# 5l1v3r1/PBS

Hardware: AMD Instinct MI355X
Metric: co-run slowdown (%) vs solo + aggregate throughput, 4-tenant mix at 1/2/4/8 GPU (higher is better)
Workload: dtype bf16

## Files before the change

csrc/hip/common.hpp:

```cpp
#pragma once
#include <hip/hip_runtime.h>

#include <cstdint>
#include <cstdio>
#include <cstdlib>

namespace gpbs_hip {

constexpr int kXcds = 8;
constexpr int kMaxTenants = 64;
constexpr int kNumPmc = 4;
constexpr uint32_t kNoOwner = 0xFFFFFFFFu;
constexpr uint32_t kSplitBit = 0x80000000u;
constexpr uint32_t kOwnerMask = 0x7FFFFFFFu;

typedef __bf16 bf16x8 __attribute__((ext_vector_type(8)));
typedef float f32x4 __attribute__((ext_vector_type(4)));
typedef float f32x16 __attribute__((ext_vector_type(16)));
typedef unsigned int u32x4 __attribute__((ext_vector_type(4)));
typedef unsigned int u32x2 __attribute__((ext_vector_type(2)));
typedef unsigned short u16;
typedef unsigned int u32;
typedef unsigned long long u64;

// ... 88 lines not shown
    const u32 se = se_id();
    const u32* w = t->owner + kCtx * (xcc & 7) + se;
    const u32 o = (mode & GATE_DEVTABLE) ? __hip_atomic_load(w, __ATOMIC_RELAXED, __HIP_MEMORY_SCOPE_AGENT)
                                         : __hip_atomic_load(w, __ATOMIC_RELAXED, __HIP_MEMORY_SCOPE_SYSTEM);
    return (o & kOwnerMask) == me;
  }
  const u64* q = t->pair[xcc & 7];
  const u64 p01 = (mode & GATE_DEVTABLE) ? __hip_atomic_load(q, __ATOMIC_RELAXED, __HIP_MEMORY_SCOPE_AGENT)
                                         : __hip_atomic_load(q, __ATOMIC_RELAXED, __HIP_MEMORY_SCOPE_SYSTEM);
  const u32 w0 = (u32)p01, w1 = (u32)(p01 >> 32);
  const bool h0 = (w0 & kOwnerMask) == me, h1 = (w1 & kOwnerMask) == me;
  if (!(mode & GATE_SPATIAL) || (h0 && h1)) {
    if (h0 || h1) return true;
    const u64 p23 = (mode & GATE_DEVTABLE) ? __hip_atomic_load(q + 1, __ATOMIC_RELAXED, __HIP_MEMORY_SCOPE_AGENT)
                                           : __hip_atomic_load(q + 1, __ATOMIC_RELAXED, __HIP_MEMORY_SCOPE_SYSTEM);
    return (u32)p23 == me || (u32)(p23 >> 32) == me;
  }
  if (h0) return !(w0 & kSplitBit) || cu_half() == 0;
  if (h1) return !(w1 & kSplitBit) || cu_half() == 1;
  return false;
}

__device__ __forceinline__ void count(u64* cnt, u32 me, u32 xcc, u64 inst, u64 cyc, u64 refs, u64 miss) {
  if (!cnt) return;
  u64* c = cnt + ((size_t)me * kXcds + (xcc & 7)) * kNumPmc;
  if (inst) __hip_atomic_fetch_add(c + 0, inst, __ATOMIC_RELAXED, __HIP_MEMORY_SCOPE_SYSTEM);
  if (cyc) __hip_atomic_fetch_add(c + 1, cyc, __ATOMIC_RELAXED, __HIP_MEMORY_SCOPE_SYSTEM);
  if (refs) __hip_atomic_fetch_add(c + 2, refs, __ATOMIC_RELAXED, __HIP_MEMORY_SCOPE_SYSTEM);
  if (miss) __hip_atomic_fetch_add(c + 3, miss, __ATOMIC_RELAXED, __HIP_MEMORY_SCOPE_SYSTEM);
}
// ... 40 lines not shown
```

csrc/hip/runtime.cpp:

```cpp
#include <hip/hip_runtime.h>
#include <hsa/hsa.h>
#include <hsa/hsa_ext_amd.h>
#include <rocprofiler-sdk-roctx/roctx.h>
#include <x86intrin.h>

#include <algorithm>
#include <atomic>
#include <cmath>
#include <cstdio>
#include <cstdlib>
#include <chrono>
#include <condition_variable>
#include <cstring>
#include <deque>
#include <memory>
#include <mutex>
#include <thread>
#include <vector>

#include "../include/gpbs/gpbs.h"
#include "common.hpp"
#include "hwc_attr.h"

using namespace gpbs_hip;

extern "C" {
int gpbs_adapt_update(gpbs_adapt_state_t*, const gpbs_adapt_params_t*, uint64_t, uint64_t, uint64_t, uint64_t);
int gpbs_hip_gemm_units(int, int);
int gpbs_hip_gemm_fp8_units(int, int);
int gpbs_hwc_sample(uint64_t* out, int nxcd);
int gpbs_hwc_sample_se(uint64_t* se_out, uint64_t* x_out);
int gpbs_hwc_slot_per_se(int k);
int gpbs_hwc_active(void);
int gpbs_hip_gemm_bf16(const void*, const void*, void*, int, int, int, void*, const void*, unsigned, unsigned, void*,
                       void*, int, hipStream_t);
int gpbs_hip_gemm_fp8(const void*, const float*, const void*, const float*, void*, int, int, int, int, void*, const void*,
                      unsigned, unsigned, void*, void*, int, hipStream_t);
int gpbs_hip_stream_copy(const void*, void*, unsigned long long, unsigned, void*, const void*, unsigned, unsigned,
                         void*, void*, int, hipStream_t);
int gpbs_hip_reduce_bf16(const void*, const void*, void*, unsigned long long, unsigned, void*, const void*, unsigned,
                         unsigned, void*, void*, int, hipStream_t);
int gpbs_hip_gemv_bf16(const void*, const void*, void*, int, int, void*, const void*, unsigned, unsigned, void*, void*,
                       int, hipStream_t);
int gpbs_hip_partition_switch(void*, unsigned, const unsigned*, hipStream_t);
int gpbs_hip_counter_reduce(void*, void*, const int*, int, void*, hipStream_t);
int gpbs_hip_adapt(void*, const void*, const void*, const void*, int, const gpbs_adapt_params_t*, int*, hipStream_t);
int gpbs_hip_switch_probe(const void*, int, unsigned*, int, unsigned, unsigned long long, hipStream_t);
int gpbs_hip_hwc_attribute(const void*, void*, void*, void*, hipStream_t);
// ... 1128 lines not shown
        (!B || X.gen > B->gen))
      B = &X;
  if (!B) return -22;
  if (hipEventQuery(B->ev) != hipSuccess) {
    B->state = 2;
    c->async_late++;
    return -11;
  }
  std::memcpy(states_out, B->st, sizeof(gpbs_adapt_state_t) * max);
  std::memcpy(tenants_out, B->ids, sizeof(int) * max);
  B->state = 0;
  return max;
}


enum Kind { K_GEMM = 1, K_STREAM = 2, K_REDUCE = 3, K_GEMV = 4, K_ALLREDUCE = 5, K_GEMM_FP8 = 6 };

constexpr int kCollMax = 8;
struct CollDescHost {
  const void* in[kCollMax];
  void* out[kCollMax];
  u32* flags[kCollMax];
  u32 rank, world;
  u64 n8;
};

struct Coll {
  int device = 0, rank = 0, world = 1;
  size_t bytes = 0;
  void* in = nullptr;
// ... 6 lines not shown

}

extern "C" {

typedef struct gpbs_runner_cfg {
  int kind;
  int tenant;
  int gate;
  int priority;
  int depth;
  int grid;
  int M, N, K;
  int chunk_bytes;
  int engine_wake;
  int reserved;
  unsigned long long bytes;
  void *a, *b, *c;
  int alt_kind;
  int alt_M, alt_N, alt_K;
  int alt_chunk_bytes;
  int alt_reserved;
  unsigned long long alt_bytes;
  void *alt_a, *alt_b, *alt_c;
} gpbs_runner_cfg_t;

typedef struct gpbs_runner_stats {
  uint64_t units_done, launches, relaunches, waits_owner, submitted;
  int64_t busy_ns, wait_owner_ns, first_start_ns, last_done_ns;
  int64_t lat_sum_ns, lat_max_ns;
  uint64_t lat_count;
// ... 233 lines not shown
  std::vector<int64_t> lats;
  hipEvent_t ev[16];
  int err = 0;
  uint64_t q_hold[16] = {};

  void hold_drop(int qi) {
    if (q_hold[qi]) {
      hold_release(ctx, q_hold[qi] - 1);
      q_hold[qi] = 0;
    }
  }

  std::atomic<int> phase{0};
  uint8_t q_alt[16] = {};
  int cur_alt = 0;
  u32 q_seq[16] = {};
  u32 coll_seq = 0;
  int64_t q_t0[16] = {};

  struct Work {
    int kind, M, N, K, chunk;
    unsigned long long bytes;
    void *a, *b, *c;
  };
  static int coll_timeout_ms(const Work& w) { return w.K > 0 ? w.K : 5000; }
  Work work(int alt) const {
    if (alt && cfg.alt_kind)
      return Work{cfg.alt_kind, cfg.alt_M, cfg.alt_N, cfg.alt_K, cfg.alt_chunk_bytes, cfg.alt_bytes,
                  cfg.alt_a, cfg.alt_b, cfg.alt_c};
    return Work{cfg.kind, cfg.M, cfg.N, cfg.K, cfg.chunk_bytes, cfg.bytes, cfg.a, cfg.b, cfg.c};
  }

  static u32 unit_total(const Work& w) {
    switch (w.kind) {
      case K_ALLREDUCE: {
        const u64 n8 = w.bytes / 16, chunk8 = (u64)w.chunk / 16, per = (n8 + w.M - 1) / w.M;
        const u64 lo = (u64)w.N * per, hi = std::min(lo + per, n8);
        return hi > lo ? (u32)((hi - lo + chunk8 - 1) / chunk8) : 0u;
      }
      case K_GEMM: return (u32)gpbs_hip_gemm_units(w.M, w.N);
// ... 90 lines not shown
    const bool dev = tm != 0;
    const void* tab = tm == 1 ? (const void*)ctx->d_table : tm == 2 ? (const void*)ctx->b_table : (const void*)ctx->h_table;
    const bool gate = cfg.gate && !ctx->share.load(std::memory_order_acquire);
    const bool hold = gate && ctx->hold_enable && tm != 1 && w.kind != K_GEMV && ctx->engine &&
                      ctx->cls_cache[cfg.tenant].load(std::memory_order_relaxed) == 1;
    const unsigned mode = (gate ? (cfg.gate == 2 ? GATE_PARK : GATE_TABLE) : GATE_NONE) | (dev ? GATE_DEVTABLE : 0) |
                          (gate && ctx->spatial ? GATE_SPATIAL : 0) |
                          (gate && __atomic_load_n(&ctx->se_mode, __ATOMIC_ACQUIRE) ? GATE_SE : 0) |
                          (cfg.priority > 0 && ctx->waveprio ? GATE_WAVEPRIO : 0) | (hold ? GATE_HOLD : 0);
    const unsigned me = (unsigned)cfg.tenant;
    __atomic_store_n(&h_status[qi], 0u, __ATOMIC_RELEASE);
    st.launches++;
    const int grid = cfg.grid ? cfg.grid : cur_grid;
    switch (w.kind) {
      case K_GEMM:
        return gpbs_hip_gemm_bf16(w.a, w.b, w.c, w.M, w.N, w.K, q, tab, mode, me, ctx->d_cnt, &h_status[qi], grid,
                                  stream);
      case K_GEMM_FP8: {
        const char *aq = (const char*)w.a, *bq = (const char*)w.b;
        return gpbs_hip_gemm_fp8(aq, (const float*)(aq + (size_t)w.M * w.K), bq, (const float*)(bq + (size_t)w.N * w.K),
                                 w.c, w.M, w.N, w.K, 0, q, tab, mode, me, ctx->d_cnt, &h_status[qi], grid, stream);
      }
      case K_STREAM:
        return gpbs_hip_stream_copy(w.a, w.c, w.bytes, (unsigned)w.chunk, q, tab, mode, me, ctx->d_cnt,
                                    &h_status[qi], grid, stream);
      case K_REDUCE:
        return gpbs_hip_reduce_bf16(w.a, w.b, w.c, w.bytes, (unsigned)w.chunk, q, tab, mode, me, ctx->d_cnt,
                                    &h_status[qi], grid, stream);
      case K_GEMV:
        return gpbs_hip_gemv_bf16(w.a, w.b, w.c, w.M, w.K, q, tab, mode, me, ctx->d_cnt, &h_status[qi], grid,
                                  stream);
      case K_ALLREDUCE:
// ... 13 lines not shown

  int wo_qi = -1;
  int64_t q_l0[16] = {};
  int64_t drain_seen_rv = 0;
  int64_t ramp_from = 0;
  static void ewma(std::atomic<int64_t>& a, std::atomic<uint64_t>& n, int64_t v) {
    const int64_t o = a.load(std::memory_order_relaxed);
    a.store(n.load(std::memory_order_relaxed) ? o + (v - o) / 8 : v, std::memory_order_relaxed);
    n.fetch_add(1, std::memory_order_relaxed);
  }
  void note_drain(int qi, int64_t now) {
    if (cfg.tenant < 0 || cfg.tenant >= kMaxTenants) return;
    const int64_t rv = ctx->revoke_ns[cfg.tenant].load(std::memory_order_relaxed);
    if (!rv || rv == drain_seen_rv || rv < q_l0[qi] || now < rv) return;
    const u32 s = __atomic_load_n(&h_status[qi], __ATOMIC_ACQUIRE);
    if ((s & 0x80000000u) && (s & 0x3fffffffu) >= unit_total(work(q_alt[qi]))) return;
    drain_seen_rv = rv;
    const int64_t dr = now - rv;
    if (dr >= 1000000000) return;
    st.drain_sum_ns += dr;
    st.drain_count++;
    if (dr > st.drain_max_ns) st.drain_max_ns = dr;
    ewma(ctx->swc_drain_ns[cfg.tenant], ctx->swc_drain_n[cfg.tenant], dr);
  }
  void note_ramp(int64_t now) {
    if (!ramp_from || cfg.tenant < 0 || cfg.tenant >= kMaxTenants) return;
    const int64_t g = ctx->grant_ns[cfg.tenant].load(std::memory_order_relaxed);
    if (g >= ramp_from && now >= g && now - g < 1000000000)
      ewma(ctx->swc_ramp_ns[cfg.tenant], ctx->swc_ramp_n[cfg.tenant], now - g);
    ramp_from = 0;
  }
// ... 66 lines not shown
            if (qi < 0) break;
            fresh = true;
          }
          wo_qi = fl.empty() ? -1 : fl.front().qi;
          wait_owner();
          if (stop) break;
          if (fresh) {
            q_alt[qi] = (uint8_t)(cfg.alt_kind && phase.load(std::memory_order_acquire));
            q_seq[qi] = coll_seq++;
            q_t0[qi] = mono_ns();
          }
          cur_alt = q_alt[qi];
          hipStream_t stream = pick_stream();
          if (fresh) {
            std::lock_guard<std::mutex> g(mu);
            pending--;
            inflight++;
            next_q = (qi + 1) % nq;
            q_busy[qi] = 1;
          } else {
            relaunch.pop_front();
            st.relaunches++;
          }
          if (cfg.priority > 0 && ctx->hold_enable && fresh && !q_hold[qi]) q_hold[qi] = hold_acquire(ctx) + 1;
          q_l0[qi] = mono_ns();
          note_ramp(q_l0[qi]);
          if (launch(qi, stream) != 0) err = -5;
          const int e = qi;
          hipEventRecord(ev[e], stream);
          fl.push_back({qi, e});
        }
        if (fl.empty()) {
          std::lock_guard<std::mutex> g(mu);
          if (pending <= 0 && relaunch.empty()) break;
          continue;
        }
        Fl f = fl.front();
        fl.pop_front();
        while (hipEventQuery(ev[f.ev]) == hipErrorNotReady) {
          if (stop) break;
          std::this_thread::yield();
        }
        const u32 s = __atomic_load_n(&h_status[f.qi], __ATOMIC_ACQUIRE);
        const u32 done = s & 0x3fffffffu;
        const Work fw = work(q_alt[f.qi]);
        const bool unfinished = !((s & 0x80000000u) && done >= unit_total(fw));
        const bool coll_late = fw.kind == K_ALLREDUCE && unfinished &&
                               mono_ns() - q_t0[f.qi] > (int64_t)coll_timeout_ms(fw) * 1000000;
        if (((s & 0x80000000u) && (s & 0x40000000u)) || coll_late) {
          std::fprintf(stderr, "[gpbs-hip] tenant %d: collective unit %u timed out waiting for its peers\n",
                       cfg.tenant, q_seq[f.qi]);
          err = -110;
          hold_drop(f.qi);
          std::lock_guard<std::mutex> g(mu);
          q_busy[f.qi] = 0;
          inflight--;
          pending = 0;
          if (!submit_times.empty()) submit_times.pop_front();
        } else if ((s & 0x80000000u) && done >= unit_total(work(q_alt[f.qi]))) {
          hold_drop(f.qi);
          const int64_t t = mono_ns();
          std::lock_guard<std::mutex> g(mu);
          q_busy[f.qi] = 0;
          inflight--;
          st.units_done++;
          st.units_alt += q_alt[f.qi];
          st.last_done_ns = t;
          if (!submit_times.empty()) {
            const int64_t lat = t - submit_times.front();
            submit_times.pop_front();
            st.lat_sum_ns += lat;
            st.lat_count++;
            if (lat > st.lat_max_ns) st.lat_max_ns = lat;
            if (lats.size() < (1u << 20)) lats.push_back(lat);
          }
        } else {
          relaunch.push_back(f.qi);
          note_drain(f.qi, mono_ns());
        }
        if (stop) break;
      }
      st.busy_ns += mono_ns() - batch_t0;
      {
// ... 1377 lines not shown
      (cfg->alt_bytes % 16 || cfg->alt_chunk_bytes <= 0 || cfg->alt_chunk_bytes % 16))
    return nullptr;
  if (cfg->alt_kind == K_GEMV && cfg->alt_K % 512) return nullptr;
  if (cfg->alt_kind == K_GEMM_FP8 &&
      (cfg->alt_M <= 0 || cfg->alt_N <= 0 || cfg->alt_K <= 0 || cfg->alt_M % 128 || cfg->alt_N % 128 || cfg->alt_K % 128))
    return nullptr;
  if (cfg->alt_kind < 0 || (cfg->alt_kind > K_GEMV && cfg->alt_kind != K_GEMM_FP8)) return nullptr;
  hipSetDevice(c->device);
  for (int have = c->cnt_rows.load(); have < cfg->tenant + 1 && !c->cnt_rows.compare_exchange_weak(have, cfg->tenant + 1);) {
  }
  auto* r = new Runner;
  r->ctx = c;
  r->cfg = *cfg;
  if (r->cfg.depth <= 0) r->cfg.depth = 2;
  if (r->cfg.depth > 8) r->cfg.depth = 8;
  r->nq = r->cfg.depth + 1;
  int lo = 0, hi = 0;
  hipDeviceGetStreamPriorityRange(&lo, &hi);
  bool ok = hipStreamCreateWithPriority(&r->stream, hipStreamNonBlocking, cfg->priority ? hi : lo) == hipSuccess;
  ok = ok && hipMalloc((void**)&r->d_q, sizeof(WorkQueue) * r->nq) == hipSuccess;
  ok = ok && hipMemset(r->d_q, 0, sizeof(WorkQueue) * r->nq) == hipSuccess;
  ok = ok && hipHostMalloc((void**)&r->h_status, sizeof(u32) * r->nq, hipHostMallocCoherent | hipHostMallocMapped) ==
                 hipSuccess;
  for (int i = 0; i < r->nq && ok; ++i) ok = hipEventCreateWithFlags(&r->ev[i], hipEventDisableTiming) == hipSuccess;
  if (!ok) {
    delete r;
    return nullptr;
  }
  r->th = std::thread([r] { r->loop(); });
  return r;
}

int gpbs_runner_submit(void* p, int units) {
  Runner* r = (Runner*)p;
  const int64_t t = mono_ns();
  {
    std::lock_guard<std::mutex> g(r->mu);
    r->pending += units;
    r->st.submitted += units;
    for (int i = 0; i < units; ++i) r->submit_times.push_back(t);
  }
  r->cv.notify_all();
  return 0;
}

// ... 377 lines not shown
```

csrc/hip/tenant_kernels.hip:

```cpp
#include "common.hpp"

namespace gpbs_hip {


__device__ __forceinline__ int grab_unit_x(WorkQueue* q, const PartTable* table, u32 mode, u32 me, u32 xcc,
                                           int* s_slot, u32 total) {
  if (threadIdx.x == 0) {
    int u = -1;
    hold_wait(table, mode);
    const u32 per = (total + kXcds - 1) / kXcds;
    for (u32 spins = 0;; ++spins) {
      if (owns(table, mode, me, xcc)) {
        for (u32 k = 0; k < (u32)kXcds; ++k) {
          const u32 r = (xcc + k) & (kXcds - 1);
          const u32 lo = r * per, hi = min(lo + per, total);
          if (lo >= hi) continue;
          if (__hip_atomic_load(&q->xnext[r], __ATOMIC_RELAXED, __HIP_MEMORY_SCOPE_AGENT) >= hi - lo) continue;
          const u32 t = atomicAdd(&q->xnext[r], 1u);
          if (t < hi - lo) {
            u = (int)(lo + t);
            atomicAdd(&q->next, 1u);
            break;
          }
        }
// ... 128 lines not shown
constexpr u32 kGemmBlock2D = 1u << 17;
constexpr u32 kGemmStatic = 1u << 18;
constexpr int kGemmOptsLive = 1 | 8 | 1 << 23;
constexpr int kGemmOptsShipped = 256 | 8192 | 65536 | 131072;
static int g_gemm_opts = 8;
constexpr int kG2Half = 128 * 128;
constexpr int kG2Buf = 4 * kG2Half;
constexpr int kG2Lds = 2 * kG2Buf;

__device__ __forceinline__ int g2_swz(int r) { return (r >> 1) & 7; }

__global__ __launch_bounds__(G2_NT, 1) void k_gemm256_bf16_tn(const u16* __restrict__ A, const u16* __restrict__ Bt,
                                                             u16* __restrict__ C, int M, int N, int K, WorkQueue* q,
                                                             const PartTable* table, u32 mode, u32 me, u64* cnt,
                                                             u32 inst_per_tile, u32 refs_per_tile, u32 miss_per_tile,
                                                             u32* status) {
  __shared__ __attribute__((aligned(16))) char smem[kG2Lds + 16];
  lds_t* lds = (lds_t*)smem;
  int* s_slot = (int*)(smem + kG2Lds);
  const u32 xcc = xcc_id();
  u64 t_last = __builtin_amdgcn_s_memtime();
  const int tid = threadIdx.x, lane = tid & 63, wid = tid >> 6;
  const int wu = __builtin_amdgcn_readfirstlane(wid);
  const int wr = wu >> 2, wc = wu & 3;
  const int tiles_m = M / G2_BM, tiles_n = N / G2_BM, ntiles = tiles_m * tiles_n;
  const int nt = K / G2_BK;
  int soff[2];
#pragma unroll
  for (int j = 0; j < 2; ++j) {
    const int row = 8 * (2 * wid + j) + (lane >> 3);
    soff[j] = row * K + (((lane & 7) ^ g2_swz(row)) * 8);
  }
  int soffa[4];
#pragma unroll
  for (int j = 0; j < 4; ++j) {
    const int row = 8 * (4 * (wid & 3) + j) + (lane >> 3);
    soffa[j] = row * K + (((lane & 7) ^ g2_swz(row)) * 8);
  }
  const int l16 = lane & 15, lq = lane >> 4;
  const int bh = wc >> 1, bc = (wc & 1) * 64;
  int units_seen = 0;

  for (;;) {
    const int tile = (mode & kGemmStatic) ? (units_seen ? -1 : (int)blockIdx.x)
                     : (mode & kGemmXRange) ? grab_unit_x(q, table, mode, me, xcc, s_slot, (u32)ntiles)
                                            : grab_unit(q, table, mode, me, xcc, s_slot, (u32)ntiles);
    if (tile < 0) break;
    int tm = tile / tiles_n, tn = tile % tiles_n;
    if ((mode & kGemmBlock2D) && (tiles_m & 3) == 0 && (tiles_n & 1) == 0 && ntiles % kXcds == 0) {
      const int per = ntiles / kXcds;
      const int bm = tiles_m / 4, bn = tiles_n / 2;
      const int g = (mode & kGemmXRange) ? tile / per : tile % kXcds;
      const int jj = (mode & kGemmXRange) ? tile % per : tile / kXcds;
      tm = (g >> 1) * bm + jj / bn;
      tn = (g & 1) * bn + jj % bn;
    }
    const u16* Ab = A + (size_t)tm * G2_BM * K;
    const u16* Bb = Bt + (size_t)tn * G2_BM * K;
    auto stage = [&](int kind, int h, int t) {
      const u16* src = (kind ? Bb : Ab) + (size_t)h * 128 * K + t * G2_BK;
      lds_t* dst = lds + (t & 1) * kG2Buf + (kind * 2 + h) * kG2Half + wid * 2048;
      glds16(src + soff[0], dst);
// ... 8 lines not shown
    auto frag = [&](int b, int kind, int h, int r0, int s) -> bf16x8 {
      const int r = r0 + l16;
      const lds_t* p = lds + b * kG2Buf + (kind * 2 + h) * kG2Half + r * 128 + (((4 * s + lq) ^ g2_swz(r)) << 4);
      return *(const __attribute__((address_space(3))) bf16x8*)p;
    };
    f32x4 acc[8][4];
#pragma unroll
    for (int i = 0; i < 8; ++i)
#pragma unroll
      for (int j = 0; j < 4; ++j) acc[i][j] = f32x4{0.f, 0.f, 0.f, 0.f};
    stage(1, 0, 0); stage(1, 1, 0); stage(0, 0, 0); stage(0, 1, 0);
    asm volatile("s_waitcnt vmcnt(0)" ::: "memory");
    __builtin_amdgcn_s_barrier();
    if (wr == 1) __builtin_amdgcn_s_barrier();
    bf16x8 a[4][2], b[4][2];
    for (int t = 0; t < nt; ++t) {
      const int buf = t & 1;
      const bool more = t + 1 < nt;
#pragma unroll
      for (int j = 0; j < 4; ++j)
#pragma unroll
        for (int s2 = 0; s2 < 2; ++s2) b[j][s2] = frag(buf, 1, bh, bc + j * 16, s2);
      __builtin_amdgcn_sched_barrier(0);
#pragma unroll
      for (int i = 0; i < 4; ++i)
#pragma unroll
        for (int s2 = 0; s2 < 2; ++s2) a[i][s2] = frag(buf, 0, wr, i * 16, s2);
      if (more) {
        stage(1, 0, t + 1); stage(1, 1, t + 1);
      } else {
        asm volatile("s_waitcnt vmcnt(0)" ::: "memory");
      }
      __builtin_amdgcn_s_barrier();
      asm volatile("s_waitcnt lgkmcnt(0)" ::: "memory");
      __builtin_amdgcn_s_setprio(1);
#pragma unroll
      for (int s2 = 0; s2 < 2; ++s2)
#pragma unroll
        for (int i = 0; i < 4; ++i)
#pragma unroll
          for (int j = 0; j < 4; ++j)
            acc[i][j] = __builtin_amdgcn_mfma_f32_16x16x32_bf16(b[j][s2], a[i][s2], acc[i][j], 0, 0, 0);
      __builtin_amdgcn_s_setprio(0);
      __builtin_amdgcn_s_barrier();
#pragma unroll
      for (int i = 0; i < 4; ++i)
// ... 3 lines not shown
        stage_own_a(t + 1);
        asm volatile("s_waitcnt vmcnt(4)" ::: "memory");
      }
      __builtin_amdgcn_s_barrier();
      asm volatile("s_waitcnt lgkmcnt(0)" ::: "memory");
      __builtin_amdgcn_s_setprio(1);
#pragma unroll
      for (int s2 = 0; s2 < 2; ++s2)
#pragma unroll
        for (int i = 0; i < 4; ++i)
#pragma unroll
          for (int j = 0; j < 4; ++j)
            acc[4 + i][j] = __builtin_amdgcn_mfma_f32_16x16x32_bf16(b[j][s2], a[i][s2], acc[4 + i][j], 0, 0, 0);
      __builtin_amdgcn_s_setprio(0);
      asm volatile("s_waitcnt vmcnt(0)" ::: "memory");
      __builtin_amdgcn_s_barrier();
    }
    if (wr == 0) __builtin_amdgcn_s_barrier();
#pragma unroll
    for (int i = 0; i < 8; ++i)
#pragma unroll
      for (int j = 0; j < 4; ++j) {
        const int m = wr * 128 + i * 16 + l16;
        const int c8 = wc * 16 + j * 4 + lq;
        const u32 lo = (u32)f2bf(acc[i][j][0]) | ((u32)f2bf(acc[i][j][1]) << 16);
        const u32 hi = (u32)f2bf(acc[i][j][2]) | ((u32)f2bf(acc[i][j][3]) << 16);
        *(__attribute__((address_space(3))) u32x2*)(lds + m * 512 + ((c8 ^ (m & 15)) << 3)) = u32x2{lo, hi};
      }
    __syncthreads();
#pragma unroll
    for (int p = 0; p < 16; ++p) {
      const int row = p * 16 + (tid >> 5), c16 = tid & 31;
      u32x4 v = *(const __attribute__((address_space(3))) u32x4*)(lds + row * 512 + (((2 * c16) ^ (row & 14)) << 3));
      if (row & 1) v = u32x4{v.z, v.w, v.x, v.y};
      u32x4* dst = (u32x4*)(C + (size_t)(tm * G2_BM + row) * N + tn * G2_BM + c16 * 8);
      __builtin_nontemporal_store(v, dst);
    }
    __syncthreads();
    ++units_seen;
    if (!(mode & kGemmStatic)) count_unit(cnt, me, xcc, inst_per_tile, &t_last, refs_per_tile, miss_per_tile, q);
  }
  if (!(mode & kGemmStatic)) finish(q, status, (u32)ntiles);
}

constexpr int SNT = 256, SUNROLL = 16, RUNROLL = 6;

template <int U, bool NTS>
__global__ __launch_bounds__(SNT) void k_stream_copy(const f32x4* __restrict__ src, f32x4* __restrict__ dst,
                                                    u64 n4, u32 chunk4, WorkQueue* q, const PartTable* table, u32 mode,
                                                    u32 me, u64* cnt, u32* status) {
  __shared__ int s_slot[4];
  const u32 xcc = xcc_id();
  u64 t_last = __builtin_amdgcn_s_memtime();
  const u32 nchunks = (u32)((n4 + chunk4 - 1) / chunk4);
  const u64 lines = (u64)chunk4 * 16 / 128;
  const u64 inst = (u64)chunk4 * 2 / 64 + 8;
  for (;;) {
// ... 175 lines not shown
    warned = true;
    fprintf(stderr,
            "gpbs_hip_set_gemm_opts: bits 0x%x select GEMM variants that were removed (docs/gemm_lab.md); "
            "the shipped schedule runs\n",
            gone);
  }
  g_gemm_opts = opts & kGemmOptsLive;
  return old;
}

int gpbs_hip_gemm_units(int M, int N) {
  if (M % G2_BM == 0 && N % G2_BM == 0) return (M / G2_BM) * (N / G2_BM);
  return (M / GBM) * (N / GBN);
}

int gpbs_hip_gemm_bf16(const void* A, const void* Bt, void* C, int M, int N, int K, void* q, const void* table,
                       unsigned mode, unsigned me, void* cnt, void* status, int grid, hipStream_t s) {
  if (M % GBM || N % GBN || K % GBK || M <= 0 || N <= 0 || K <= 0) return -22;
  if (M % G2_BM == 0 && N % G2_BM == 0) {
    const int ntiles = (M / G2_BM) * (N / G2_BM);
    if (grid <= 0) grid = 256;
    if (grid > ntiles) grid = ntiles;
    const u32 inst = (u32)((G2_BM / 16) * (G2_BM / 16) * (K / 32) + (K / G2_BK) * 64 + 128);
    const u32 refs = (u32)(((u64)2 * G2_BM * K * 2) / 128);
    const u32 miss = (u32)((((u64)M + N) * K * 2 / 128) / ntiles + (u64)G2_BM * G2_BM * 2 / 128);
    const u32 m2 = mode | ((g_gemm_opts & 1) ? kGemmXRange : 0u) |
                   ((g_gemm_opts & 8) && ntiles % kXcds == 0 ? kGemmBlock2D : 0u) |
                   ((g_gemm_opts & (1 << 23)) && (mode & 3) == GATE_NONE && grid == ntiles ? kGemmStatic : 0u);
    hipLaunchKernelGGL(k_gemm256_bf16_tn, dim3(grid), dim3(G2_NT), 0, s, (const u16*)A, (const u16*)Bt, (u16*)C, M, N,
                       K, (WorkQueue*)q, (const PartTable*)table, m2, me, (u64*)cnt, inst, refs, miss, (u32*)status);
    return hipGetLastError() == hipSuccess ? 0 : -5;
  }
  const int ntiles = (M / GBM) * (N / GBN);
  if (grid <= 0) grid = 256 * 2;
  if (grid > ntiles) grid = ntiles;
  const u32 inst = (u32)((GBM / 16) * (GBN / 16) * (K / 32) * 2 + (K / GBK) * 32 + 64);
  const u32 refs = (u32)(((u64)(GBM + GBN) * K * 2) / 128);
  const u32 miss = (u32)((((u64)M + N) * K * 2 / 128) / ntiles + (u64)GBM * GBN * 2 / 128);
  hipLaunchKernelGGL(k_gemm_bf16_tn, dim3(grid), dim3(GNT), 0, s, (const u16*)A, (const u16*)Bt, (u16*)C, M, N, K,
                     (WorkQueue*)q, (const PartTable*)table, mode, me, (u64*)cnt, inst, refs, miss, (u32*)status);
  return hipGetLastError() == hipSuccess ? 0 : -5;
}

static int g_stream_opts = 0;

int gpbs_hip_set_stream_opts(int opts) {
  const int old = g_stream_opts;
  if (opts >= 0) g_stream_opts = opts;
  return old;
}

int gpbs_hip_stream_copy(const void* src, void* dst, unsigned long long bytes, unsigned chunk_bytes, void* q,
                         const void* table, unsigned mode, unsigned me, void* cnt, void* status, int grid, hipStream_t s) {
  if (bytes % 16 || chunk_bytes % 16 || chunk_bytes == 0) return -22;
  if (grid <= 0) grid = 256;
  using K = void (*)(const f32x4*, f32x4*, u64, u32, WorkQueue*, const PartTable*, u32, u32, u64*, u32*);
// ... 50 lines not shown
```

pbs_amd/ops/hipabi.py:

```python
from __future__ import annotations

import ctypes as C

from .. import _native as N

u32, i32, u64, i64 = C.c_uint32, C.c_int32, C.c_uint64, C.c_int64
vp = C.c_void_p


class RunnerCfg(C.Structure):
    _fields_ = [(n, C.c_int) for n in ("kind", "tenant", "gate", "priority", "depth", "grid", "M", "N", "K",
                                       "chunk_bytes", "engine_wake", "reserved")] + \
               [("bytes", C.c_ulonglong), ("a", vp), ("b", vp), ("c", vp)] + \
               [(n, C.c_int) for n in ("alt_kind", "alt_M", "alt_N", "alt_K", "alt_chunk_bytes", "alt_reserved")] + \
               [("alt_bytes", C.c_ulonglong), ("alt_a", vp), ("alt_b", vp), ("alt_c", vp)]


class RunnerStats(C.Structure):
    _fields_ = [(n, u64) for n in ("units_done", "launches", "relaunches", "waits_owner", "submitted")] + \
               [(n, i64) for n in ("busy_ns", "wait_owner_ns", "first_start_ns", "last_done_ns", "lat_sum_ns",
                                   "lat_max_ns")] + [("lat_count", u64), ("units_alt", u64)] + \
               [("drain_sum_ns", i64), ("drain_max_ns", i64), ("drain_count", u64)]


KIND = {"gemm": 1, "stream": 2, "reduce": 3, "gemv": 4, "allreduce": 5, "gemm_fp8": 6}


def _p(lib, name, res, *args):
    f = getattr(lib, name)
    f.restype = res
    f.argtypes = list(args)


def bind(lib):
    _p(lib, "gpbs_roctx_push", C.c_int, C.c_char_p)
    _p(lib, "gpbs_roctx_pop", C.c_int)
    _p(lib, "gpbs_roctx_mark", None, C.c_char_p)
    _p(lib, "gpbs_gpu_switch_latency", C.c_int, vp, C.c_int, C.c_int, vp)
    _p(lib, "gpbs_hip_gemm_bf16", C.c_int, vp, vp, vp, C.c_int, C.c_int, C.c_int, vp, vp, C.c_uint, C.c_uint, vp, vp,
       C.c_int, vp)
    _p(lib, "gpbs_hip_gemm_fp8", C.c_int, vp, vp, vp, vp, vp, C.c_int, C.c_int, C.c_int, C.c_int, vp, vp, C.c_uint,
       C.c_uint, vp, vp, C.c_int, vp)
    _p(lib, "gpbs_hip_gemm_fp8_units", C.c_int, C.c_int, C.c_int)
    _p(lib, "gpbs_hip_stream_copy", C.c_int, vp, vp, C.c_ulonglong, C.c_uint, vp, vp, C.c_uint, C.c_uint, vp, vp,
       C.c_int, vp)
    _p(lib, "gpbs_hip_reduce_bf16", C.c_int, vp, vp, vp, C.c_ulonglong, C.c_uint, vp, vp, C.c_uint, C.c_uint, vp, vp,
       C.c_int, vp)
    _p(lib, "gpbs_hip_gemv_bf16", C.c_int, vp, vp, vp, C.c_int, C.c_int, vp, vp, C.c_uint, C.c_uint, vp, vp, C.c_int,
       vp)
    _p(lib, "gpbs_hip_set_gemm_opts", C.c_int, C.c_int)
    _p(lib, "gpbs_hip_set_reduce_opts", C.c_int, C.c_int)
    _p(lib, "gpbs_hip_set_stream_opts", C.c_int, C.c_int)
    _p(lib, "gpbs_hwc_init", C.c_int, C.c_char_p)
    _p(lib, "gpbs_hwc_init_gpu", C.c_int, C.c_char_p, C.c_int)
    _p(lib, "gpbs_hwc_start", C.c_int)
# ... 75 lines not shown
    _p(lib, "gpbs_hip_hwc_attr_bench", C.c_int, C.c_int, C.POINTER(C.c_double))
    _p(lib, "gpbs_hip_adapt_pools_selftest", C.c_int, C.c_int)
    _p(lib, "gpbs_gpu_ctx_destroy", None, vp)
    _p(lib, "gpbs_gpu_attach", C.c_int, vp, vp, C.c_int, C.c_int)
    _p(lib, "gpbs_gpu_backend_ops", C.c_int, vp, vp, C.POINTER(N.ActuatorOps), C.POINTER(N.CounterOps), C.c_int)
    _p(lib, "gpbs_gpu_table", vp, vp)
    _p(lib, "gpbs_gpu_counters", vp, vp)
    _p(lib, "gpbs_gpu_set_owners", C.c_int, vp, C.POINTER(C.c_int))
    _p(lib, "gpbs_gpu_get_owners", C.c_int, vp, C.POINTER(C.c_int))
    _p(lib, "gpbs_gpu_read_counters", C.c_int, vp, C.c_int, C.POINTER(u64), C.POINTER(u64))
    _p(lib, "gpbs_gpu_stats", C.c_int, vp, C.POINTER(u64))
    _p(lib, "gpbs_gpu_ownership", C.c_int, vp, C.c_int, C.POINTER(i64), C.c_int)
    _p(lib, "gpbs_gpu_cumask_stream", vp, C.c_int, C.POINTER(C.c_uint32), C.c_int, C.c_int)
    _p(lib, "gpbs_gpu_stream_destroy", C.c_int, vp)
    _p(lib, "gpbs_runner_create", vp, vp, C.POINTER(RunnerCfg))
    _p(lib, "gpbs_runner_submit", C.c_int, vp, C.c_int)
    _p(lib, "gpbs_runner_wait", C.c_int, vp, i64)
    _p(lib, "gpbs_runner_stats", C.c_int, vp, C.POINTER(RunnerStats))
    _p(lib, "gpbs_runner_latencies", C.c_int, vp, C.POINTER(i64), C.c_int, C.c_int)
    _p(lib, "gpbs_runner_reset_stats", C.c_int, vp)
    _p(lib, "gpbs_runner_set_gate", C.c_int, vp, C.c_int)
    _p(lib, "gpbs_runner_cancel", i64, vp)
    _p(lib, "gpbs_runner_set_engine_wake", C.c_int, vp, C.c_int)
    _p(lib, "gpbs_runner_stream", vp, vp)
    _p(lib, "gpbs_runner_set_phase", C.c_int, vp, C.c_int)
    _p(lib, "gpbs_coll_create", vp, C.c_int, C.c_int, C.c_int, C.c_ulonglong)
    _p(lib, "gpbs_coll_export", C.c_int, vp, vp)
    _p(lib, "gpbs_coll_handle_bytes", C.c_int)
    _p(lib, "gpbs_coll_open", C.c_int, vp, C.c_int, vp)
    _p(lib, "gpbs_coll_finalize", C.c_int, vp)
# ... 14 lines not shown
```

pbs_amd/runtime/gpu.py:

```python
from __future__ import annotations

import ctypes as C
import os
from dataclasses import dataclass
from typing import Dict, List, Optional

os.environ["GPU_MAX_HW_QUEUES"] = os.environ.get("GPBS_HWQ") or str(max(12, int(os.environ.get("GPU_MAX_HW_QUEUES", "0") or 0)))

import torch

from .. import _native as N
from ..ops import hipabi
from ..ops.kernels import lib as hiplib

XCDS = 8
CTX = 4


class GpuContext:
    def __init__(self, device: int = 0, engine=None, part_base: int = 0, table_mode: str = "host",
                 device_counters: bool = True, device_adapt: bool = False, nctx: int = 1,
                 params: Optional[Dict[str, int]] = None):
        self.L = hiplib()
        self.device = device
# ... 277 lines not shown
    wait_owner_ns: int
    first_start_ns: int
    last_done_ns: int
    lat_sum_ns: int
    lat_max_ns: int
    lat_count: int
    units_alt: int = 0
    drain_sum_ns: int = 0
    drain_max_ns: int = 0
    drain_count: int = 0


class Runner:

    def __init__(self, ctx: GpuContext, kind: str, tenant: int, *, gate: bool = True, priority: int = 0,
                 depth: int = 2, grid: int = 0, engine_wake: bool = True, alt: Optional[dict] = None, **shape):
        self.ctx = ctx
        self.L = ctx.L
        self.kind = kind
        self.tenant = tenant
        dev = torch.device("cuda", ctx.device)
        g = torch.Generator(device=dev)
        g.manual_seed(1234 + tenant)
        cfg = hipabi.RunnerCfg()
        cfg.tenant = tenant
        cfg.gate = int(gate)
        cfg.priority = priority
        cfg.depth = depth
        cfg.grid = grid
        cfg.engine_wake = int(engine_wake)
        self.buffers = []
        w = self._workload(kind, shape, dev, g)
        cfg.kind, cfg.M, cfg.N, cfg.K, cfg.chunk_bytes, cfg.bytes = w["kind"], w["M"], w["N"], w["K"], w["chunk"], w["bytes"]
        cfg.a, cfg.b, cfg.c = w["a"], w["b"], w["c"]
        self.work_per_unit, self.unit_name = w["work"], w["unit"]
        self.alt_kind = None
        if alt:
            alt = dict(alt)
            self.alt_kind = alt.pop("kind")
            v = self._workload(self.alt_kind, alt, dev, g)
            cfg.alt_kind, cfg.alt_M, cfg.alt_N, cfg.alt_K = v["kind"], v["M"], v["N"], v["K"]
            cfg.alt_chunk_bytes, cfg.alt_bytes = v["chunk"], v["bytes"]
            cfg.alt_a, cfg.alt_b, cfg.alt_c = v["a"], v["b"], v["c"]
            self.alt_work_per_unit = v["work"]
        torch.cuda.synchronize(dev)
# ... 124 lines not shown
```

Measured before the change: 1.260.

## Batch multiple GEMM units per launch and prefetch next tile ticket during K loop

Low-priority GEMM runners now pack up to a configurable batch of pending units into a single persistent-kernel launch. The kernel's tile queue spans n copies of the tile grid, and the host accounting scales completion checks and latency bookkeeping by the batch count. Inside the kernel, the ownership table read is issued early and the next tile ticket is claimed during the last K iteration, which overlaps queue atomics with compute and epilogue. This cuts per-launch overhead and grab latency, at the cost of coarser preemption granularity and redundant writes to the same C buffer.

```diff
diff --git a/csrc/hip/common.hpp b/csrc/hip/common.hpp
--- a/csrc/hip/common.hpp
+++ b/csrc/hip/common.hpp
@@ -126,6 +126,43 @@
     if (h0 || h1) return true;
     const u64 p23 = (mode & GATE_DEVTABLE) ? __hip_atomic_load(q + 1, __ATOMIC_RELAXED, __HIP_MEMORY_SCOPE_AGENT)
                                            : __hip_atomic_load(q + 1, __ATOMIC_RELAXED, __HIP_MEMORY_SCOPE_SYSTEM);
+    return (u32)p23 == me || (u32)(p23 >> 32) == me;
+  }
+  if (h0) return !(w0 & kSplitBit) || cu_half() == 0;
+  if (h1) return !(w1 & kSplitBit) || cu_half() == 1;
+  return false;
+}
+
+struct OwnWords {
+  u32 se;
+  u64 p01;
+};
+
+__device__ __forceinline__ OwnWords own_issue(const PartTable* t, u32 mode, u32 xcc) {
+  OwnWords w;
+  if ((mode & 3) == GATE_NONE) return w;
+  if (mode & GATE_SE) {
+    const u32* p = t->owner + kCtx * (xcc & 7) + se_id();
+    w.se = (mode & GATE_DEVTABLE) ? __hip_atomic_load(p, __ATOMIC_RELAXED, __HIP_MEMORY_SCOPE_AGENT)
+                                  : __hip_atomic_load(p, __ATOMIC_RELAXED, __HIP_MEMORY_SCOPE_SYSTEM);
+    return w;
+  }
+  const u64* q = t->pair[xcc & 7];
+  w.p01 = (mode & GATE_DEVTABLE) ? __hip_atomic_load(q, __ATOMIC_RELAXED, __HIP_MEMORY_SCOPE_AGENT)
+                                 : __hip_atomic_load(q, __ATOMIC_RELAXED, __HIP_MEMORY_SCOPE_SYSTEM);
+  return w;
+}
+
+__device__ __forceinline__ bool own_decide(const OwnWords w, const PartTable* t, u32 mode, u32 me, u32 xcc) {
+  if ((mode & 3) == GATE_NONE) return true;
+  if (mode & GATE_SE) return (w.se & kOwnerMask) == me;
+  const u32 w0 = (u32)w.p01, w1 = (u32)(w.p01 >> 32);
+  const bool h0 = (w0 & kOwnerMask) == me, h1 = (w1 & kOwnerMask) == me;
+  if (!(mode & GATE_SPATIAL) || (h0 && h1)) {
+    if (h0 || h1) return true;
+    const u64* q = t->pair[xcc & 7] + 1;
+    const u64 p23 = (mode & GATE_DEVTABLE) ? __hip_atomic_load(q, __ATOMIC_RELAXED, __HIP_MEMORY_SCOPE_AGENT)
+                                           : __hip_atomic_load(q, __ATOMIC_RELAXED, __HIP_MEMORY_SCOPE_SYSTEM);
     return (u32)p23 == me || (u32)(p23 >> 32) == me;
   }
   if (h0) return !(w0 & kSplitBit) || cu_half() == 0;
diff --git a/csrc/hip/runtime.cpp b/csrc/hip/runtime.cpp
--- a/csrc/hip/runtime.cpp
+++ b/csrc/hip/runtime.cpp
@@ -32,6 +32,8 @@
 int gpbs_hwc_sample_se(uint64_t* se_out, uint64_t* x_out);
 int gpbs_hwc_slot_per_se(int k);
 int gpbs_hwc_active(void);
+int gpbs_hip_gemm_bf16_n(const void*, const void*, void*, int, int, int, int, void*, const void*, unsigned, unsigned,
+                         void*, void*, int, hipStream_t);
 int gpbs_hip_gemm_bf16(const void*, const void*, void*, int, int, int, void*, const void*, unsigned, unsigned, void*,
                        void*, int, hipStream_t);
 int gpbs_hip_gemm_fp8(const void*, const float*, const void*, const float*, void*, int, int, int, int, void*, const void*,
@@ -1190,6 +1192,8 @@
 }
 
 
+constexpr int kGemmBatchDefault = 4;
+constexpr int kGemmBatchMax = 64;
 enum Kind { K_GEMM = 1, K_STREAM = 2, K_REDUCE = 3, K_GEMV = 4, K_ALLREDUCE = 5, K_GEMM_FP8 = 6 };
 
 constexpr int kCollMax = 8;
@@ -1226,7 +1230,7 @@
   int M, N, K;
   int chunk_bytes;
   int engine_wake;
-  int reserved;
+  int batch;
   unsigned long long bytes;
   void *a, *b, *c;
   int alt_kind;
@@ -1490,6 +1494,7 @@
   std::atomic<int> phase{0};
   uint8_t q_alt[16] = {};
   int cur_alt = 0;
+  int q_n[16] = {};
   u32 q_seq[16] = {};
   u32 coll_seq = 0;
   int64_t q_t0[16] = {};
@@ -1500,6 +1505,10 @@
     void *a, *b, *c;
   };
   static int coll_timeout_ms(const Work& w) { return w.K > 0 ? w.K : 5000; }
+  int batch_for(const Work& w) const {
+    if (w.kind != K_GEMM || cfg.priority != 0 || w.M % 256 || w.N % 256) return 1;
+    return cfg.batch > 0 ? cfg.batch : kGemmBatchDefault;
+  }
   Work work(int alt) const {
     if (alt && cfg.alt_kind)
       return Work{cfg.alt_kind, cfg.alt_M, cfg.alt_N, cfg.alt_K, cfg.alt_chunk_bytes, cfg.alt_bytes,
@@ -1620,8 +1629,8 @@
     const int grid = cfg.grid ? cfg.grid : cur_grid;
     switch (w.kind) {
       case K_GEMM:
-        return gpbs_hip_gemm_bf16(w.a, w.b, w.c, w.M, w.N, w.K, q, tab, mode, me, ctx->d_cnt, &h_status[qi], grid,
-                                  stream);
+        return gpbs_hip_gemm_bf16_n(w.a, w.b, w.c, w.M, w.N, w.K, q_n[qi], q, tab, mode, me, ctx->d_cnt, &h_status[qi],
+                                    grid, stream);
       case K_GEMM_FP8: {
         const char *aq = (const char*)w.a, *bq = (const char*)w.b;
         return gpbs_hip_gemm_fp8(aq, (const float*)(aq + (size_t)w.M * w.K), bq, (const float*)(bq + (size_t)w.N * w.K),
@@ -1665,7 +1674,7 @@
     const int64_t rv = ctx->revoke_ns[cfg.tenant].load(std::memory_order_relaxed);
     if (!rv || rv == drain_seen_rv || rv < q_l0[qi] || now < rv) return;
     const u32 s = __atomic_load_n(&h_status[qi], __ATOMIC_ACQUIRE);
-    if ((s & 0x80000000u) && (s & 0x3fffffffu) >= unit_total(work(q_alt[qi]))) return;
+    if ((s & 0x80000000u) && (s & 0x3fffffffu) >= (u32)q_n[qi] * unit_total(work(q_alt[qi]))) return;
     drain_seen_rv = rv;
     const int64_t dr = now - rv;
     if (dr >= 1000000000) return;
@@ -1762,8 +1771,10 @@
           hipStream_t stream = pick_stream();
           if (fresh) {
             std::lock_guard<std::mutex> g(mu);
-            pending--;
-            inflight++;
+            q_n[qi] = (int)std::min<int64_t>(pending, batch_for(work(cur_alt)));
+            if (q_n[qi] < 1) q_n[qi] = 1;
+            pending -= q_n[qi];
+            inflight += q_n[qi];
             next_q = (qi + 1) % nq;
             q_busy[qi] = 1;
           } else {
@@ -1792,7 +1803,7 @@
         const u32 s = __atomic_load_n(&h_status[f.qi], __ATOMIC_ACQUIRE);
         const u32 done = s & 0x3fffffffu;
         const Work fw = work(q_alt[f.qi]);
-        const bool unfinished = !((s & 0x80000000u) && done >= unit_total(fw));
+        const bool unfinished = !((s & 0x80000000u) && done >= (u32)q_n[f.qi] * unit_total(fw));
         const bool coll_late = fw.kind == K_ALLREDUCE && unfinished &&
                                mono_ns() - q_t0[f.qi] > (int64_t)coll_timeout_ms(fw) * 1000000;
         if (((s & 0x80000000u) && (s & 0x40000000u)) || coll_late) {
@@ -1802,19 +1813,19 @@
           hold_drop(f.qi);
           std::lock_guard<std::mutex> g(mu);
           q_busy[f.qi] = 0;
-          inflight--;
+          inflight -= q_n[f.qi];
           pending = 0;
-          if (!submit_times.empty()) submit_times.pop_front();
-        } else if ((s & 0x80000000u) && done >= unit_total(work(q_alt[f.qi]))) {
+          for (int k = 0; k < q_n[f.qi] && !submit_times.empty(); ++k) submit_times.pop_front();
+        } else if (!unfinished) {
           hold_drop(f.qi);
           const int64_t t = mono_ns();
           std::lock_guard<std::mutex> g(mu);
           q_busy[f.qi] = 0;
-          inflight--;
-          st.units_done++;
-          st.units_alt += q_alt[f.qi];
+          inflight -= q_n[f.qi];
+          st.units_done += (uint64_t)q_n[f.qi];
+          st.units_alt += (uint64_t)q_alt[f.qi] * (uint64_t)q_n[f.qi];
           st.last_done_ns = t;
-          if (!submit_times.empty()) {
+          for (int k = 0; k < q_n[f.qi] && !submit_times.empty(); ++k) {
             const int64_t lat = t - submit_times.front();
             submit_times.pop_front();
             st.lat_sum_ns += lat;
@@ -3222,6 +3233,8 @@
   r->cfg = *cfg;
   if (r->cfg.depth <= 0) r->cfg.depth = 2;
   if (r->cfg.depth > 8) r->cfg.depth = 8;
+  if (r->cfg.batch < 0) r->cfg.batch = 1;
+  if (r->cfg.batch > kGemmBatchMax) r->cfg.batch = kGemmBatchMax;
   r->nq = r->cfg.depth + 1;
   int lo = 0, hi = 0;
   hipDeviceGetStreamPriorityRange(&lo, &hi);
@@ -3237,6 +3250,11 @@
   }
   r->th = std::thread([r] { r->loop(); });
   return r;
+}
+
+int gpbs_runner_cfg_layout(int* batch_offset) {
+  if (batch_offset) *batch_offset = (int)offsetof(gpbs_runner_cfg_t, batch);
+  return (int)sizeof(gpbs_runner_cfg_t);
 }
 
 int gpbs_runner_submit(void* p, int units) {
diff --git a/csrc/hip/tenant_kernels.hip b/csrc/hip/tenant_kernels.hip
--- a/csrc/hip/tenant_kernels.hip
+++ b/csrc/hip/tenant_kernels.hip
@@ -166,7 +166,7 @@
                                                              u16* __restrict__ C, int M, int N, int K, WorkQueue* q,
                                                              const PartTable* table, u32 mode, u32 me, u64* cnt,
                                                              u32 inst_per_tile, u32 refs_per_tile, u32 miss_per_tile,
-                                                             u32* status) {
+                                                             u32* status, u32 nunits) {
   __shared__ __attribute__((aligned(16))) char smem[kG2Lds + 16];
   lds_t* lds = (lds_t*)smem;
   int* s_slot = (int*)(smem + kG2Lds);
@@ -177,6 +177,7 @@
   const int wr = wu >> 2, wc = wu & 3;
   const int tiles_m = M / G2_BM, tiles_n = N / G2_BM, ntiles = tiles_m * tiles_n;
   const int nt = K / G2_BK;
+  const u32 total = nunits * (u32)ntiles;
   int soff[2];
 #pragma unroll
   for (int j = 0; j < 2; ++j) {
@@ -192,12 +193,17 @@
   const int l16 = lane & 15, lq = lane >> 4;
   const int bh = wc >> 1, bc = (wc & 1) * 64;
   int units_seen = 0;
+  const bool prefetch = !(mode & (GATE_HOLD | kGemmXRange | kGemmStatic));
+  constexpr int kNoTicket = -2;
+  int tile = kNoTicket;
 
   for (;;) {
-    const int tile = (mode & kGemmStatic) ? (units_seen ? -1 : (int)blockIdx.x)
-                     : (mode & kGemmXRange) ? grab_unit_x(q, table, mode, me, xcc, s_slot, (u32)ntiles)
-                                            : grab_unit(q, table, mode, me, xcc, s_slot, (u32)ntiles);
+    if (tile == kNoTicket)
+      tile = (mode & kGemmStatic) ? (units_seen ? -1 : (int)blockIdx.x)
+             : (mode & kGemmXRange) ? grab_unit_x(q, table, mode, me, xcc, s_slot, (u32)ntiles)
+                                    : grab_unit(q, table, mode, me, xcc, s_slot, total);
     if (tile < 0) break;
+    if (nunits > 1) tile %= ntiles;
     int tm = tile / tiles_n, tn = tile % tiles_n;
     if ((mode & kGemmBlock2D) && (tiles_m & 3) == 0 && (tiles_n & 1) == 0 && ntiles % kXcds == 0) {
       const int per = ntiles / kXcds;
@@ -236,6 +242,9 @@
     __builtin_amdgcn_s_barrier();
     if (wr == 1) __builtin_amdgcn_s_barrier();
     bf16x8 a[4][2], b[4][2];
+    OwnWords own;
+    u32 ticket;
+    bool claimed = false;
     for (int t = 0; t < nt; ++t) {
       const int buf = t & 1;
       const bool more = t + 1 < nt;
@@ -252,6 +261,7 @@
         stage(1, 0, t + 1); stage(1, 1, t + 1);
       } else {
         asm volatile("s_waitcnt vmcnt(0)" ::: "memory");
+        if (prefetch && tid == 0) own = own_issue(table, mode, xcc);
       }
       __builtin_amdgcn_s_barrier();
       asm volatile("s_waitcnt lgkmcnt(0)" ::: "memory");
@@ -285,6 +295,12 @@
             acc[4 + i][j] = __builtin_amdgcn_mfma_f32_16x16x32_bf16(b[j][s2], a[i][s2], acc[4 + i][j], 0, 0, 0);
       __builtin_amdgcn_s_setprio(0);
       asm volatile("s_waitcnt vmcnt(0)" ::: "memory");
+      if (prefetch && !more && tid == 0 && own_decide(own, table, mode, me, xcc)) {
+        u32 zero = 0;
+        asm volatile("" : "+v"(zero));
+        ticket = __hip_atomic_fetch_add(&q->next + zero, 1u, __ATOMIC_RELAXED, __HIP_MEMORY_SCOPE_AGENT);
+        claimed = true;
+      }
       __builtin_amdgcn_s_barrier();
     }
     if (wr == 0) __builtin_amdgcn_s_barrier();
@@ -298,7 +314,10 @@
         const u32 hi = (u32)f2bf(acc[i][j][2]) | ((u32)f2bf(acc[i][j][3]) << 16);
         *(__attribute__((address_space(3))) u32x2*)(lds + m * 512 + ((c8 ^ (m & 15)) << 3)) = u32x2{lo, hi};
       }
-    __syncthreads();
+    asm volatile("s_waitcnt lgkmcnt(0)" ::: "memory");
+    __builtin_amdgcn_s_barrier();
+    asm volatile("" ::"v"(ticket));
+    if (prefetch && tid == 0) s_slot[1] = claimed ? (ticket < total ? (int)ticket : -1) : kNoTicket;
 #pragma unroll
     for (int p = 0; p < 16; ++p) {
       const int row = p * 16 + (tid >> 5), c16 = tid & 31;
@@ -308,10 +327,11 @@
       __builtin_nontemporal_store(v, dst);
     }
     __syncthreads();
+    tile = prefetch ? s_slot[1] : kNoTicket;
     ++units_seen;
     if (!(mode & kGemmStatic)) count_unit(cnt, me, xcc, inst_per_tile, &t_last, refs_per_tile, miss_per_tile, q);
   }
-  if (!(mode & kGemmStatic)) finish(q, status, (u32)ntiles);
+  if (!(mode & kGemmStatic)) finish(q, status, total);
 }
 
 constexpr int SNT = 256, SUNROLL = 16, RUNROLL = 6;
@@ -517,9 +537,12 @@
   return (M / GBM) * (N / GBN);
 }
 
-int gpbs_hip_gemm_bf16(const void* A, const void* Bt, void* C, int M, int N, int K, void* q, const void* table,
-                       unsigned mode, unsigned me, void* cnt, void* status, int grid, hipStream_t s) {
-  if (M % GBM || N % GBN || K % GBK || M <= 0 || N <= 0 || K <= 0) return -22;
+int gpbs_hip_gemm_bf16_n(const void* A, const void* Bt, void* C, int M, int N, int K, int n, void* q,
+                         const void* table, unsigned mode, unsigned me, void* cnt, void* status, int grid,
+                         hipStream_t s) {
+  if (M % GBM || N % GBN || K % GBK || M <= 0 || N <= 0 || K <= 0 || n < 1) return -22;
+  if (n > 1 && (M % G2_BM || N % G2_BM || (g_gemm_opts & 1) || (long long)n * (M / G2_BM) * (N / G2_BM) >= 1 << 30))
+    return -22;
   if (M % G2_BM == 0 && N % G2_BM == 0) {
     const int ntiles = (M / G2_BM) * (N / G2_BM);
     if (grid <= 0) grid = 256;
@@ -529,9 +552,10 @@
     const u32 miss = (u32)((((u64)M + N) * K * 2 / 128) / ntiles + (u64)G2_BM * G2_BM * 2 / 128);
     const u32 m2 = mode | ((g_gemm_opts & 1) ? kGemmXRange : 0u) |
                    ((g_gemm_opts & 8) && ntiles % kXcds == 0 ? kGemmBlock2D : 0u) |
-                   ((g_gemm_opts & (1 << 23)) && (mode & 3) == GATE_NONE && grid == ntiles ? kGemmStatic : 0u);
+                   ((g_gemm_opts & (1 << 23)) && (mode & 3) == GATE_NONE && grid == ntiles && n == 1 ? kGemmStatic : 0u);
     hipLaunchKernelGGL(k_gemm256_bf16_tn, dim3(grid), dim3(G2_NT), 0, s, (const u16*)A, (const u16*)Bt, (u16*)C, M, N,
-                       K, (WorkQueue*)q, (const PartTable*)table, m2, me, (u64*)cnt, inst, refs, miss, (u32*)status);
+                       K, (WorkQueue*)q, (const PartTable*)table, m2, me, (u64*)cnt, inst, refs, miss, (u32*)status,
+                       (u32)n);
     return hipGetLastError() == hipSuccess ? 0 : -5;
   }
   const int ntiles = (M / GBM) * (N / GBN);
@@ -543,6 +567,11 @@
   hipLaunchKernelGGL(k_gemm_bf16_tn, dim3(grid), dim3(GNT), 0, s, (const u16*)A, (const u16*)Bt, (u16*)C, M, N, K,
                      (WorkQueue*)q, (const PartTable*)table, mode, me, (u64*)cnt, inst, refs, miss, (u32*)status);
   return hipGetLastError() == hipSuccess ? 0 : -5;
+}
+
+int gpbs_hip_gemm_bf16(const void* A, const void* Bt, void* C, int M, int N, int K, void* q, const void* table,
+                       unsigned mode, unsigned me, void* cnt, void* status, int grid, hipStream_t s) {
+  return gpbs_hip_gemm_bf16_n(A, Bt, C, M, N, K, 1, q, table, mode, me, cnt, status, grid, s);
 }
 
 static int g_stream_opts = 0;
diff --git a/pbs_amd/ops/hipabi.py b/pbs_amd/ops/hipabi.py
--- a/pbs_amd/ops/hipabi.py
+++ b/pbs_amd/ops/hipabi.py
@@ -10,7 +10,7 @@
 
 class RunnerCfg(C.Structure):
     _fields_ = [(n, C.c_int) for n in ("kind", "tenant", "gate", "priority", "depth", "grid", "M", "N", "K",
-                                       "chunk_bytes", "engine_wake", "reserved")] + \
+                                       "chunk_bytes", "engine_wake", "batch")] + \
                [("bytes", C.c_ulonglong), ("a", vp), ("b", vp), ("c", vp)] + \
                [(n, C.c_int) for n in ("alt_kind", "alt_M", "alt_N", "alt_K", "alt_chunk_bytes", "alt_reserved")] + \
                [("alt_bytes", C.c_ulonglong), ("alt_a", vp), ("alt_b", vp), ("alt_c", vp)]
@@ -39,6 +39,8 @@
     _p(lib, "gpbs_gpu_switch_latency", C.c_int, vp, C.c_int, C.c_int, vp)
     _p(lib, "gpbs_hip_gemm_bf16", C.c_int, vp, vp, vp, C.c_int, C.c_int, C.c_int, vp, vp, C.c_uint, C.c_uint, vp, vp,
        C.c_int, vp)
+    _p(lib, "gpbs_hip_gemm_bf16_n", C.c_int, vp, vp, vp, C.c_int, C.c_int, C.c_int, C.c_int, vp, vp, C.c_uint, C.c_uint,
+       vp, vp, C.c_int, vp)
     _p(lib, "gpbs_hip_gemm_fp8", C.c_int, vp, vp, vp, vp, vp, C.c_int, C.c_int, C.c_int, C.c_int, vp, vp, C.c_uint,
        C.c_uint, vp, vp, C.c_int, vp)
     _p(lib, "gpbs_hip_gemm_fp8_units", C.c_int, C.c_int, C.c_int)
@@ -144,6 +146,7 @@
     _p(lib, "gpbs_gpu_cumask_stream", vp, C.c_int, C.POINTER(C.c_uint32), C.c_int, C.c_int)
     _p(lib, "gpbs_gpu_stream_destroy", C.c_int, vp)
     _p(lib, "gpbs_runner_create", vp, vp, C.POINTER(RunnerCfg))
+    _p(lib, "gpbs_runner_cfg_layout", C.c_int, C.POINTER(C.c_int))
     _p(lib, "gpbs_runner_submit", C.c_int, vp, C.c_int)
     _p(lib, "gpbs_runner_wait", C.c_int, vp, i64)
     _p(lib, "gpbs_runner_stats", C.c_int, vp, C.POINTER(RunnerStats))
diff --git a/pbs_amd/runtime/gpu.py b/pbs_amd/runtime/gpu.py
--- a/pbs_amd/runtime/gpu.py
+++ b/pbs_amd/runtime/gpu.py
@@ -315,7 +315,8 @@
 class Runner:
 
     def __init__(self, ctx: GpuContext, kind: str, tenant: int, *, gate: bool = True, priority: int = 0,
-                 depth: int = 2, grid: int = 0, engine_wake: bool = True, alt: Optional[dict] = None, **shape):
+                 depth: int = 2, grid: int = 0, engine_wake: bool = True, alt: Optional[dict] = None,
+                 batch: int = 0, **shape):
         self.ctx = ctx
         self.L = ctx.L
         self.kind = kind
@@ -330,6 +331,7 @@
         cfg.depth = depth
         cfg.grid = grid
         cfg.engine_wake = int(engine_wake)
+        cfg.batch = batch
         self.buffers = []
         w = self._workload(kind, shape, dev, g)
         cfg.kind, cfg.M, cfg.N, cfg.K, cfg.chunk_bytes, cfg.bytes = w["kind"], w["M"], w["N"], w["K"], w["chunk"], w["bytes"]
```

New measurement: 1.237. -1.9%, worse.
